# funcwj/setk

Measured on AMD Instinct MI355X. Metric: real-time-factor (audio-sec/wall-sec), 8-ch 16 kHz MVDR, higher is better.
Workload: dtype f32; 1 GPU; 8-ch 16 kHz oracle-mask MVDR, 30 s utterances, 125 per GPU (BASELINE configs[2] shard: 1000 at 8 GPUs), STFT 512/256/hann/center, inputs resident in HBM; utts_per_gpu=125, channels=8, frames=1876, beamformer=mvdr, parallelism=utterance-sharded x1

## Files before the change

setk_amd/csrc/pass2_mc.hip:

```cpp
#include "common.h"
#include "fft512.h"
#include "mcdft.h"
#include <cstdio>
#include <cstdlib>
#include <type_traits>

namespace setk {

constexpr int kP2McWavesPerSimd = 4;
constexpr int kP2McGroup = 2;
constexpr int p2mc_threads(bool pcm) { return pcm ? 1024 : 512; }

constexpr int kP2McTiles = 25;
size_t pass2_mc_lds_bytes(int C, bool pcm) {
    const size_t nw = p2mc_threads(pcm) / 64;
    const size_t wt = ((size_t)C * kBins * sizeof(cf) + 15) & ~(size_t)15;
    return wt + kP2McTiles * 1024 + 2048 + nw * kP2McGroup * 8 * mc::kOddPitch * sizeof(float) +
           nw * kP2McGroup * 16 * sizeof(float) + 64 + (pcm ? nw * C * 64 * sizeof(uint2) : 0);
}

SETK_DEV float row8_sum(float x) {
    int v = __builtin_bit_cast(int, x);
    x += __builtin_bit_cast(float, __builtin_amdgcn_update_dpp(0, v, 0xB1, 0xf, 0xf, true));
    v = __builtin_bit_cast(int, x);
    x += __builtin_bit_cast(float, __builtin_amdgcn_update_dpp(0, v, 0x4E, 0xf, 0xf, true));
    v = __builtin_bit_cast(int, x);
    x += __builtin_bit_cast(float, __builtin_amdgcn_update_dpp(0, v, 0x141, 0xf, 0xf, true));
    return x;
}
SETK_DEV float wave_max_nonneg(float x) {
    int v = __builtin_bit_cast(int, x);
    x = fmaxf(x, __builtin_bit_cast(float, __builtin_amdgcn_update_dpp(0, v, 0xB1, 0xf, 0xf, true)));
    v = __builtin_bit_cast(int, x);
    x = fmaxf(x, __builtin_bit_cast(float, __builtin_amdgcn_update_dpp(0, v, 0x4E, 0xf, 0xf, true)));
    v = __builtin_bit_cast(int, x);
    x = fmaxf(x, __builtin_bit_cast(float, __builtin_amdgcn_update_dpp(0, v, 0x141, 0xf, 0xf, true)));
    v = __builtin_bit_cast(int, x);
    x = fmaxf(x, __builtin_bit_cast(float, __builtin_amdgcn_update_dpp(0, v, 0x140, 0xf, 0xf, true)));
    const unsigned b = __builtin_bit_cast(unsigned, x);
    unsigned m = __builtin_amdgcn_readlane(b, 0);
    const unsigned m1 = __builtin_amdgcn_readlane(b, 16), m2 = __builtin_amdgcn_readlane(b, 32),
                   m3 = __builtin_amdgcn_readlane(b, 48);
    m = m > m1 ? m : m1;
    m = m > m2 ? m : m2;
    m = m > m3 ? m : m3;
    return __builtin_bit_cast(float, m);
}

template <int C, bool PCM = false>
__global__ __launch_bounds__(p2mc_threads(PCM), kP2McWavesPerSimd) void beamform_istft_mc_kernel(Pass2Args a) {
    constexpr int NT = p2mc_threads(PCM);
    constexpr int NW = NT / 64;
    constexpr int F = kBins;

    extern __shared__ __attribute__((aligned(16))) char smem[];
    char* p = smem;
    cf* wtab = reinterpret_cast<cf*>(p);
    p += ((size_t)C * F * sizeof(cf) + 15) & ~(size_t)15;
    mc::u4* tiles = reinterpret_cast<mc::u4*>(p);
    p += kP2McTiles * 1024;
    mc::f4* synr = reinterpret_cast<mc::f4*>(p);
    p += 2048;
    float* a16s = reinterpret_cast<float*>(p);
    p += (size_t)NW * kP2McGroup * 8 * mc::kOddPitch * sizeof(float);
    float* yodd_s = reinterpret_cast<float*>(p);
    p += NW * kP2McGroup * 16 * sizeof(float);
    float* red = reinterpret_cast<float*>(p);
    p += 64;
    uint2* carry_s = reinterpret_cast<uint2*>(p);

    const int tid = threadIdx.x;
    const int lane = tid & 63;
    const int wave = __builtin_amdgcn_readfirstlane(tid >> 6);
    const int c16 = lane & 15, g = lane >> 4;
    const WorkItem wi = a.items[blockIdx.x];
    const UttDesc ud = a.utts[wi.utt];
    const int n_samp = ud.num_samples;
    const int T = ud.num_frames;
    const int hop = kNfft / 2;
    const bool post_mask = (a.flags & 0x4) != 0;
    const bool clamp = (a.flags & 0x2) != 0;

    float in_sc = PCM ? 3.0517578125e-05f : 1.f, out_sc = 1.f;
    if (a.norm_bits) {
        const unsigned nb = a.norm_bits[wi.utt];
        int e = (int)((nb >> 23) & 0xff) - 126;
        e = (__builtin_bit_cast(float, nb) <= 1.f) ? 0 : (e > 100 ? 100 : e);
        in_sc *= __builtin_bit_cast(float, (unsigned)(127 - e) << 23);
        out_sc = __builtin_bit_cast(float, (unsigned)(127 + e) << 23);
    }
    {
        const cf* wsrc = reinterpret_cast<const cf*>(a.weight) + (size_t)wi.utt * C * kBinsPad;
        for (int i = tid; i < C * F; i += NT) {
            const int c = i / F, f = i - c * F;
            wtab[i] = wsrc[c * kBinsPad + f];
        }
    }
    mc::stage_tiles(tiles, a.mc_tab, mc::kW_BR_H, 10, tid, NT);
    mc::stage_tiles(tiles + 10 * 64, a.mc_tab, mc::kW_OT_H, 2, tid, NT);
    mc::stage_tiles(tiles + 12 * 64, a.mc_tab, mc::kW_MC_H, 8, tid, NT);
    for (int i = tid; i < 128; i += NT) {
        const int l = i & 63, t4 = i >> 6;
        const mc::f4 w = {a.mc_win[(4 * t4 + 0) * 64 + l] * in_sc, a.mc_win[(4 * t4 + 1) * 64 + l] * in_sc,
                          a.mc_win[(4 * t4 + 2) * 64 + l] * in_sc, a.mc_win[(4 * t4 + 3) * 64 + l] * in_sc};
        tiles[20 * 64 + i] = __builtin_bit_cast(mc::u4, w);
    }
    mc::stage_tiles(tiles + 22 * 64, a.mc_tab, mc::kW_TR, 3, tid, NT);
    for (int i = tid; i < 128; i += NT) {
        const int l = i & 63, hf = i >> 6;
        synr[i] = (mc::f4){a.mc_syn[(4 * hf + 0) * 64 + l] * out_sc, a.mc_syn[(4 * hf + 1) * 64 + l] * out_sc,
                           a.mc_syn[(4 * hf + 2) * 64 + l] * out_sc, a.mc_syn[(4 * hf + 3) * 64 + l] * out_sc};
    }
    struct { float tr[4], ti[4]; } K;
    float* yoddw = yodd_s + wave * kP2McGroup * 16;
    const int lane_bin = mc::bin_of(c16, g, 0);
    const cf* wl = wtab + lane_bin;
    const int lane_n = 64 * g + c16;
    float omax = 0.f;
    __syncthreads();

    const int per = (wi.t1 - wi.t0 + NW - 1) / NW;
    const int ta = wi.t0 + wave * per;
    const int tb = min(ta + per, wi.t1);
    const int tw = ta > 0 ? ta - 1 : ta;

    constexpr int R = kP2McGroup;
    float* a16g = a16s + wave * R * 8 * mc::kOddPitch;
    float carry[4] = {0.f, 0.f, 0.f, 0.f};
    auto chan = [&](int c) {
        if constexpr (PCM) return (gcshort_p)gptr(ud.audio) + (size_t)c * ud.ch_stride;
        else return gptr(ud.audio) + (size_t)c * n_samp;
    };
    uint2* carry_l = carry_s + (size_t)wave * C * 64 + lane;
    auto load_pair = [&](float (&v)[12], int (&nr)[4], int t0, int c, auto edge) __attribute__((always_inline)) {
        const auto x = chan(c);
        const int o = 64 * g + c16;
        const int s0 = min(t0, T - 1) * hop - a.g.pad, s1 = min(t0 + 1, T - 1) * hop - a.g.pad + 256;
        auto base = [&](int s) __attribute__((always_inline)) {
            auto xs = x + s;
            if constexpr (C > 2) asm volatile("" : "+s"(xs));
            return xs;
        };
        const auto xa = base(s0), xb = base(s1);
        auto at = [&](decltype(xa) xs, int s, int k) __attribute__((always_inline)) {
            if constexpr (C > 2) return xs + ((unsigned)o + (unsigned)k);
            else return x + (s + o + k);
        };
        if constexpr (PCM) {
            const uint2 pk = carry_l[64 * c];
            v[0] = (float)(short)(pk.x & 0xffff);
            v[1] = (float)((int)pk.x >> 16);
            v[2] = (float)(short)(pk.y & 0xffff);
            v[3] = (float)((int)pk.y >> 16);
            if (!decltype(edge)::value) {
#pragma unroll
                for (int e = 0; e < 4; ++e) {
                    v[4 + e] = *at(xa, s0, 256 + 16 * e);
                    nr[e] = *at(xb, s1, 16 * e);
                }
            } else {
#pragma unroll
                for (int e = 0; e < 4; ++e) {
                    v[4 + e] = x[reflect_index(s0 + o + 256 + 16 * e, n_samp)];
                    nr[e] = x[reflect_index(s1 + o + 16 * e, n_samp)];
                }
            }
        } else {
            if (!decltype(edge)::value) {
#pragma unroll
                for (int e = 0; e < 4; ++e) {
                    v[e] = __builtin_nontemporal_load(at(xa, s0, 16 * e));
                    v[4 + e] = __builtin_nontemporal_load(at(xa, s0, 256 + 16 * e));
                }
#pragma unroll
                for (int e = 0; e < 4; ++e) v[8 + e] = *at(xb, s1, 16 * e);
            } else {
#pragma unroll
                for (int e = 0; e < 4; ++e) {
                    v[e] = x[reflect_index(s0 + o + 16 * e, n_samp)];
                    v[4 + e] = x[reflect_index(s0 + o + 256 + 16 * e, n_samp)];
                    v[8 + e] = x[reflect_index(s1 + o + 16 * e, n_samp)];
                }
            }
        }
    };
    mc::f4 yr[R], yi[R];
    static_assert(R == 2, "the paired transform and the LDS carry are written for groups of two frames");
    constexpr bool kTwoBuf = !PCM && C >= 5;
    float buf_a[12], buf_b[12];
    int nraw_a[4], nraw_b[4];
    auto channel = [&](const float (&cur)[12], const int (&craw)[4], float (&nx)[12], int (&nxraw)[4], int t0,
                       int c, bool more, auto edge) __attribute__((always_inline)) {
        float x0[8], x1[8];
#pragma unroll
        for (int e = 0; e < 4; ++e) {
            x0[e] = cur[e];
            x0[4 + e] = cur[4 + e];
            x1[e] = cur[4 + e];
            if constexpr (PCM) x1[4 + e] = (float)craw[e];
            else x1[4 + e] = cur[8 + e];
        }
        if constexpr (PCM) {
            carry_l[64 * c] = make_uint2(__builtin_amdgcn_perm((unsigned)craw[1], (unsigned)craw[0], 0x05040100u),
                                         __builtin_amdgcn_perm((unsigned)craw[3], (unsigned)craw[2], 0x05040100u));
        }
        if (more) load_pair(nx, nxraw, t0, c + 1, edge);
        mc::f4 zr0, zi0, a16_0, zr1, zi1, a16_1;
        {
            asm volatile("" ::: "memory");
            const mc::f4 w0 = __builtin_bit_cast(mc::f4, tiles[20 * 64 + lane]);
            const mc::f4 w1 = __builtin_bit_cast(mc::f4, tiles[21 * 64 + lane]);
            const float win[8] = {w0[0], w0[1], w0[2], w0[3], w1[0], w1[1], w1[2], w1[3]};
            mc::forward2_t(x0, x1, win, [&](int i) { return mc::lds_h8(tiles, 12 + i, lane); },
                           [&](int i) { return __builtin_bit_cast(mc::f4, tiles[(22 + i) * 64 + lane]); },
                           zr0, zi0, a16_0, zr1, zi1, a16_1);
        }
        __builtin_amdgcn_sched_barrier(0);
        asm volatile("" ::: "memory");
        const cf* wc = wl + c * F;
        cf w[4];
#pragma unroll
        for (int r = 0; r < 4; ++r) w[r] = wc[32 * r];
        mc::store_a16(a16g, c, lane, a16_0);
        mc::store_a16(a16g + 8 * mc::kOddPitch, c, lane, a16_1);
#pragma unroll
        for (int r = 0; r < 4; ++r) {
            yr[0][r] = fmaf(zr0[r], w[r].x, fmaf(zi0[r], w[r].y, yr[0][r]));
            yi[0][r] = fmaf(zi0[r], w[r].x, fmaf(-zr0[r], w[r].y, yi[0][r]));
            yr[1][r] = fmaf(zr1[r], w[r].x, fmaf(zi1[r], w[r].y, yr[1][r]));
            yi[1][r] = fmaf(zi1[r], w[r].x, fmaf(-zr1[r], w[r].y, yi[1][r]));
        }
        if constexpr (kTwoBuf) {
#pragma unroll
            for (int k = 0; k < R; ++k) {
                asm volatile("" : "+v"(yr[k][0]), "+v"(yr[k][1]), "+v"(yr[k][2]), "+v"(yr[k][3]),
                                  "+v"(yi[k][0]), "+v"(yi[k][1]), "+v"(yi[k][2]), "+v"(yi[k][3]));
            }
        }
        __builtin_amdgcn_sched_barrier(0);
    };
    auto group = [&](int t0, auto edge) __attribute__((always_inline)) {
#pragma unroll
        for (int k = 0; k < R; ++k) {
            yr[k] = (mc::f4){0.f, 0.f, 0.f, 0.f};
            yi[k] = (mc::f4){0.f, 0.f, 0.f, 0.f};
        }
        if constexpr (decltype(edge)::value || !kTwoBuf) {
#pragma unroll 1
            for (int c = 0; c < C; ++c) channel(buf_a, nraw_a, buf_a, nraw_a, t0, c, c + 1 < C, edge);
        } else {
            int c = 0;
#pragma unroll 1
            for (; c + 2 < C; c += 2) {
                channel(buf_a, nraw_a, buf_b, nraw_b, t0, c, true, edge);
                channel(buf_b, nraw_b, buf_a, nraw_a, t0, c + 1, true, edge);
            }
            if constexpr (C % 2 == 0) {
                channel(buf_a, nraw_a, buf_b, nraw_b, t0, c, true, edge);
                channel(buf_b, nraw_b, buf_a, nraw_a, t0, c + 1, false, edge);
            } else {
                channel(buf_a, nraw_a, buf_b, nraw_b, t0, c, false, edge);
            }
        }
    };
    auto span_is_edge = [&](int t0) {
        const int lo = t0 * hop - a.g.pad, hi = (t0 + R - 1) * hop - a.g.pad + kNfft;
        return lo < 0 || hi > n_samp || t0 + R > T;
    };
    auto request_group = [&](int t0) __attribute__((always_inline)) {
        if (span_is_edge(t0)) load_pair(buf_a, nraw_a, t0, 0, std::true_type());
        else load_pair(buf_a, nraw_a, t0, 0, std::false_type());
    };
    if constexpr (PCM) {
        if (tw < tb) {
#pragma unroll 1
            for (int c = 0; c < C; ++c) {
                const auto x = chan(c);
                const int s0 = tw * hop - a.g.pad, o = 64 * g + c16;
                int r[4];
#pragma unroll
                for (int e = 0; e < 4; ++e) r[e] = x[reflect_index(s0 + o + 16 * e, n_samp)];
                carry_l[64 * c] = make_uint2(__builtin_amdgcn_perm((unsigned)r[1], (unsigned)r[0], 0x05040100u),
                                             __builtin_amdgcn_perm((unsigned)r[3], (unsigned)r[2], 0x05040100u));
            }
        }
    }
    if (tw < tb) request_group(tw);
#pragma unroll 1
    for (int t0 = tw; t0 < tb; t0 += R) {
        const int nf = min(R, tb - t0);
        if (span_is_edge(t0)) group(t0, std::true_type());
        else group(t0, std::false_type());
        if (t0 + R < tb) request_group(t0 + R);
        const int t1 = min(t0 + 1, T - 1);
        int lt = lane;
        asm volatile("" : "+v"(lt));
        const int kf = (lt >> 3) & 1, co = lt & 7, c16 = lt & 15, g = lt >> 4;
        const bool odd_on = co < C;
        const cf* wo = wtab + (odd_on ? co : 0) * F + 16 + 64 * g;
        const int orow = 8 * kf + (odd_on ? co : C - 1);
        float yo[4];
        {
            asm volatile("" ::: "memory");
            const mc::f4 d = mc::odd_tile_row(a16g, mc::lds_h8(tiles, 10, lane), mc::lds_h8(tiles, 11, lane), lane, orow);
            const cf w0 = wo[0], w1 = wo[32];
            yo[0] = odd_on ? fmaf(d[0], w0.x, d[1] * w0.y) : 0.f;
            yo[1] = odd_on ? fmaf(d[1], w0.x, -d[0] * w0.y) : 0.f;
            yo[2] = odd_on ? fmaf(d[2], w1.x, d[3] * w1.y) : 0.f;
            yo[3] = odd_on ? fmaf(d[3], w1.x, -d[2] * w1.y) : 0.f;
#pragma unroll
            for (int i = 0; i < 4; ++i) yo[i] = row8_sum(yo[i]);
        }
        mc::f4 fr[R], fi[R];
#pragma unroll
        for (int k = 0; k < R; ++k) {
            fr[k] = yr[k];
            fi[k] = yi[k];
        }
        if (post_mask) {
            const float* mrow = ud.mask_s + (size_t)t0 * F;
            const unsigned dm = (unsigned)(t1 - t0) * F;
            unsigned mo = (unsigned)lane_bin, mq = 16u + 64u * (unsigned)g + (kf ? dm : 0u);
            asm volatile("" : "+v"(mo), "+v"(mq));
#pragma unroll
            for (int k = 0; k < R; ++k) {
#pragma unroll
                for (int r = 0; r < 4; ++r) {
                    float m = mrow[mo + (k ? dm : 0u) + 32 * r];
                    if (clamp) m = fminf(m, 1.f);
                    fr[k][r] *= m;
                    fi[k][r] *= m;
                }
            }
            float m0 = mrow[mq], m1 = mrow[mq + 32];
            if (clamp) { m0 = fminf(m0, 1.f); m1 = fminf(m1, 1.f); }
            yo[0] *= m0;
            yo[1] *= m0;
            yo[2] *= m1;
            yo[3] *= m1;
        }
        const float yom = fmaxf(fmaxf(fabsf(yo[0]), fabsf(yo[1])), fmaxf(fabsf(yo[2]), fabsf(yo[3])));
        float sc[R], isc[R];
#pragma unroll
        for (int k = 0; k < R; ++k) {
            fi[k][0] = (lane == 0) ? 0.f : fi[k][0];
            fi[k][3] = (lane == 32) ? 0.f : fi[k][3];
            float mxl = (kf == k) ? yom : 0.f;
#pragma unroll
            for (int r = 0; r < 4; ++r) mxl = fmaxf(mxl, fmaxf(fabsf(fr[k][r]), fabsf(fi[k][r])));
            const float mxw = wave_max_nonneg(mxl);
            int ex = (int)((__builtin_bit_cast(unsigned, mxw) >> 23) & 0xff);
            ex = ex < 16 ? 16 : (ex > 250 ? 250 : ex);
            sc[k] = __builtin_bit_cast(float, (unsigned)(264 - ex) << 23);
            isc[k] = __builtin_bit_cast(float, (unsigned)(ex - 10) << 23);
        }
        {
            const float scl = kf ? sc[1] : sc[0];
            if ((c16 & 7) == 0) *reinterpret_cast<mc::f4*>(yoddw + 16 * kf + 4 * g) = (mc::f4){yo[0] * scl, yo[1] * scl, yo[2] * scl, yo[3] * scl};
        }
        float e16[R];
        {
            float v[8];
            const mc::f4 v0 = *reinterpret_cast<const mc::f4*>(yoddw + 16 * (c16 & 1) + 8 * (g & 1));
            const mc::f4 v1 = *reinterpret_cast<const mc::f4*>(yoddw + 16 * (c16 & 1) + 8 * (g & 1) + 4);
            const float rowsel = c16 < R ? 1.f : 0.f;
#pragma unroll
            for (int e = 0; e < 4; ++e) {
                v[e] = v0[e] * rowsel;
                v[4 + e] = v1[e] * rowsel;
            }
            const mc::f4 d = mc::inv_odd_tile(v, mc::lds_h8(tiles, 8, lane), mc::lds_h8(tiles, 9, lane), lane);
            e16[0] = d[0];
            e16[1] = d[1];
        }
#pragma unroll
        for (int k = 0; k < R; ++k) {
#pragma unroll
            for (int r = 0; r < 4; ++r) {
                fr[k][r] *= sc[k];
                fi[k][r] *= sc[k];
            }
        }
        float bmid0[8], bmid1[8];
        {
            const mc::f4 tt0 = __builtin_bit_cast(mc::f4, tiles[22 * 64 + lane]);
            const mc::f4 tt1 = __builtin_bit_cast(mc::f4, tiles[23 * 64 + lane]);
#pragma unroll
            for (int r = 0; r < 4; ++r) {
                K.tr[r] = tt0[r];
                K.ti[r] = tt1[r];
            }
        }
        auto inv_tile = [&](int i) { return mc::lds_h8(tiles, i, lane); };
        mc::inverse2_a(fr[0], fi[0], e16[0], fr[1], fi[1], e16[1], inv_tile, K.tr, K.ti, bmid0, bmid1, lane);
        asm volatile("" ::: "memory");
        mc::f4 y0[R], y1[R];
        mc::inverse2_b(bmid0, bmid1, inv_tile, y0[0], y1[0], y0[1], y1[1]);
        const mc::f4 s0 = synr[lane], s1 = synr[64 + lane];
#pragma unroll
        for (int k = 0; k < R; ++k) {
            if (k >= nf) break;
            const int t = t0 + k;
            float blk[4];
#pragma unroll
            for (int r = 0; r < 4; ++r) blk[r] = fmaf(y0[k][r], s0[r] * isc[k], carry[r]);
            if (t == 0) {
#pragma unroll
                for (int r = 0; r < 4; ++r) blk[r] *= gptr(a.mc_edge)[r * 64 + lane];
            }
            if (t >= ta) {
                const int o = t * hop - a.g.pad + lane_n;
#pragma unroll
                for (int r = 0; r < 4; ++r) {
                    const int oo = o + 16 * r;
                    if (oo >= 0 && oo < ud.out_len) {
                        ud.wave_f32[oo] = blk[r];
                        omax = fmaxf(omax, fabsf(blk[r]));
                    }
                }
            }
#pragma unroll
            for (int r = 0; r < 4; ++r) carry[r] = y1[k][r] * (s1[r] * isc[k]);
        }
    }
    if (tb == T && ta < tb) {
        const int o = T * hop - a.g.pad + lane_n;
#pragma unroll
        for (int r = 0; r < 4; ++r) {
            const int oo = o + 16 * r;
            const float v = carry[r] * gptr(a.mc_edge)[(4 + r) * 64 + lane];
            if (oo >= 0 && oo < ud.out_len) {
                ud.wave_f32[oo] = v;
                omax = fmaxf(omax, fabsf(v));
            }
        }
    }
#pragma unroll
    for (int o = 32; o > 0; o >>= 1) omax = fmaxf(omax, __shfl_xor(omax, o));
    if ((tid & 63) == 0) red[tid >> 6] = omax;
    __syncthreads();
    if (tid == 0) {
        float m = red[0];
#pragma unroll
        for (int w = 1; w < NT / 64; ++w) m = fmaxf(m, red[w]);
        atomicMax(a.outmax_bits + wi.utt, __float_as_uint(m));
    }
}

int pass2_mc_wgs_per_cu(int C, bool pcm) {
    const int by_waves = kP2McWavesPerSimd * 4 / (p2mc_threads(pcm) / 64);
    const int by_lds = (int)((160u << 10) / pass2_mc_lds_bytes(C, pcm));
    return by_waves < by_lds ? (by_waves > 0 ? by_waves : 1) : (by_lds > 0 ? by_lds : 1);
}

template <int C, bool PCM = false>
static hipError_t launch_pass2_mc_t(const Pass2Args& a, int n_items, hipStream_t s) {
    const size_t lds = pass2_mc_lds_bytes(C, PCM);
    auto k = beamform_istft_mc_kernel<C, PCM>;
    hipError_t e = hipFuncSetAttribute(reinterpret_cast<const void*>(k),
                                       hipFuncAttributeMaxDynamicSharedMemorySize, (int)lds);
    if (e != hipSuccess) return e;
    hipLaunchKernelGGL(k, dim3(n_items), dim3(p2mc_threads(PCM)), lds, s, a);
    return hipGetLastError();
}

hipError_t launch_pass2_mc(int C, const Pass2Args& a, int n_items, hipStream_t s, bool pcm16) {
#define SETK_CASE(c) \
    case c: return pcm16 ? launch_pass2_mc_t<c, true>(a, n_items, s) : launch_pass2_mc_t<c>(a, n_items, s);
    switch (C) {
        SETK_CASE(1)
        SETK_CASE(2)
        SETK_CASE(3)
        SETK_CASE(4)
        SETK_CASE(5)
        SETK_CASE(6)
        SETK_CASE(7)
        SETK_CASE(8)
    }
#undef SETK_CASE
    return hipErrorInvalidValue;
}

}
```

Before: 2.193 million x real time (audio seconds per wall second, all GPUs).

## Hand off overlap-add carry between waves via LDS instead of recomputing halo frame

Previously each wave other than the first recomputed the frame before its range (tw = ta-1) to build the overlap-add carry for its first output frame. Now only wave 0 uses a warm-up frame. Later waves park their first frame's first half and scale in LDS, and after a barrier take the previous wave's final carry from LDS to finish that frame. Per-wave ranges are rounded to the pair size so groups stay aligned. This removes one redundant frame of multichannel transform and beamforming per wave, at the cost of extra LDS, two block barriers and some load imbalance from the rounding.

```diff
diff --git a/setk_amd/csrc/pass2_mc.hip b/setk_amd/csrc/pass2_mc.hip
--- a/setk_amd/csrc/pass2_mc.hip
+++ b/setk_amd/csrc/pass2_mc.hip
@@ -12,11 +12,13 @@
 constexpr int p2mc_threads(bool pcm) { return pcm ? 1024 : 512; }
 
 constexpr int kP2McTiles = 25;
+constexpr int kP2McPark = 5;
 size_t pass2_mc_lds_bytes(int C, bool pcm) {
     const size_t nw = p2mc_threads(pcm) / 64;
     const size_t wt = ((size_t)C * kBins * sizeof(cf) + 15) & ~(size_t)15;
     return wt + kP2McTiles * 1024 + 2048 + nw * kP2McGroup * 8 * mc::kOddPitch * sizeof(float) +
-           nw * kP2McGroup * 16 * sizeof(float) + 64 + (pcm ? nw * C * 64 * sizeof(uint2) : 0);
+           nw * kP2McGroup * 16 * sizeof(float) + 64 + nw * kP2McPark * 64 * sizeof(float) +
+           (pcm ? nw * C * 64 * sizeof(uint2) : 0);
 }
 
 SETK_DEV float row8_sum(float x) {
@@ -67,6 +69,8 @@
     p += NW * kP2McGroup * 16 * sizeof(float);
     float* red = reinterpret_cast<float*>(p);
     p += 64;
+    float* park_s = reinterpret_cast<float*>(p);
+    p += (size_t)NW * kP2McPark * 64 * sizeof(float);
     uint2* carry_s = reinterpret_cast<uint2*>(p);
 
     const int tid = threadIdx.x;
@@ -119,10 +123,11 @@
     float omax = 0.f;
     __syncthreads();
 
-    const int per = (wi.t1 - wi.t0 + NW - 1) / NW;
+    const int per = ((wi.t1 - wi.t0 + NW - 1) / NW + kP2McGroup - 1) / kP2McGroup * kP2McGroup;
     const int ta = wi.t0 + wave * per;
     const int tb = min(ta + per, wi.t1);
-    const int tw = ta > 0 ? ta - 1 : ta;
+    const int tw = (wave == 0 && ta > 0) ? ta - 1 : ta;
+    const int te = wave > 0 ? ta + 1 : ta;
 
     constexpr int R = kP2McGroup;
     float* a16g = a16s + wave * R * 8 * mc::kOddPitch;
@@ -185,6 +190,7 @@
         }
     };
     mc::f4 yr[R], yi[R];
+    constexpr bool kParkSkips = !PCM && (C == 5 || C == 6);
     static_assert(R == 2, "the paired transform and the LDS carry are written for groups of two frames");
     constexpr bool kTwoBuf = !PCM && C >= 5;
     float buf_a[12], buf_b[12];
@@ -401,6 +407,19 @@
         for (int k = 0; k < R; ++k) {
             if (k >= nf) break;
             const int t = t0 + k;
+            if (k == 0 && wave > 0 && t0 == ta) {
+                int lp = lane;
+                asm volatile("" : "+v"(lp));
+                float* pk = park_s + wave * (kP2McPark * 64) + lp;
+#pragma unroll
+                for (int r = 0; r < 4; ++r) pk[64 * r] = y0[0][r];
+                pk[64 * 4] = isc[0];
+                if constexpr (kParkSkips) {
+#pragma unroll
+                    for (int r = 0; r < 4; ++r) carry[r] = y1[0][r] * (s1[r] * isc[0]);
+                    continue;
+                }
+            }
             float blk[4];
 #pragma unroll
             for (int r = 0; r < 4; ++r) blk[r] = fmaf(y0[k][r], s0[r] * isc[k], carry[r]);
@@ -408,7 +427,7 @@
 #pragma unroll
                 for (int r = 0; r < 4; ++r) blk[r] *= gptr(a.mc_edge)[r * 64 + lane];
             }
-            if (t >= ta) {
+            if (t >= te) {
                 const int o = t * hop - a.g.pad + lane_n;
 #pragma unroll
                 for (int r = 0; r < 4; ++r) {
@@ -432,6 +451,30 @@
             if (oo >= 0 && oo < ud.out_len) {
                 ud.wave_f32[oo] = v;
                 omax = fmaxf(omax, fabsf(v));
+            }
+        }
+    }
+    __syncthreads();
+    {
+        int lt = lane;
+        asm volatile("" : "+v"(lt));
+        mc::f4* hand = reinterpret_cast<mc::f4*>(tiles);
+        if (ta < tb) hand[wave * 64 + lt] = (mc::f4){carry[0], carry[1], carry[2], carry[3]};
+        __syncthreads();
+        if (wave > 0 && ta < tb) {
+            const mc::f4 cp = hand[(wave - 1) * 64 + lt];
+            const float* pk = park_s + wave * (kP2McPark * 64) + lt;
+            const float isc0 = pk[64 * 4];
+            const mc::f4 s0 = synr[lt];
+            const int o = ta * hop - a.g.pad + 64 * (lt >> 4) + (lt & 15);
+#pragma unroll
+            for (int r = 0; r < 4; ++r) {
+                const float blk = fmaf(pk[64 * r], s0[r] * isc0, cp[r]);
+                const int oo = o + 16 * r;
+                if (oo >= 0 && oo < ud.out_len) {
+                    ud.wave_f32[oo] = blk;
+                    omax = fmaxf(omax, fabsf(blk));
+                }
             }
         }
     }
```

Result: no change. 2.200 million x real time (audio seconds per wall second, all GPUs), median of 6 (+0.3%).
